# ParBLiSS/kmerind

Measured on AMD Instinct MI355X. Metric: kmers_per_sec_indexed, higher is better.
Workload: dtype u64

## Files before the change

kmerind_amd/csrc/kmi_superkmer.h:

```cpp
#pragma once

namespace kmi {

constexpr int kRecNShift = 38, kRecHashShift = 43;
constexpr uint64_t kSkPadW1 = ~0ull;
constexpr int kRecEdgeShift = 32;
constexpr uint32_t kSkEdgeWindows = 3;
__device__ __forceinline__ uint32_t rec_hash18(uint64_t w1) { return (uint32_t)(w1 >> kRecHashShift) & 0x3ffffu; }
__device__ __forceinline__ uint32_t rec_fine_sub(uint64_t w1) { return (rec_hash18(w1) >> 3) & 127u; }

constexpr int kSkThreads = 512;
constexpr int kSkRoundTiles = 24;
constexpr int kSkListCap = 32;

struct SkRound {
  uint64_t t; uint32_t ei, total; uint32_t eo[kSkRoundTiles + 1]; uint64_t nt; uint32_t nei;
};
__device__ __forceinline__ bool sk_plan(const uint32_t *__restrict__ ent_cnt, uint64_t te, uint64_t t, uint32_t ei, SkRound &r) {
  while (t < te && ei >= ent_cnt[t]) { ++t; ei = 0; }
  if (t >= te) return false;
  r.t = t; r.ei = ei; r.eo[0] = 0;
  r.nt = t + kSkRoundTiles; r.nei = 0;
  bool cut = false;
#pragma unroll
// ... 321 lines not shown
      if (threadIdx.x < cur.total) { sk_locate(cur, threadIdx.x, ent_stride, tr, eidx); ev = ent[eidx]; ri = run_items[eidx]; }
      cnt = ri >> 26;
      const uint32_t *src = wg_items + (ri & 0x3ffffffu);
#pragma unroll
      for (int j = 0; j < CAP; ++j) it[j] = ((uint32_t)j < cnt) ? src[j] : 0u;
      const uint64_t ip0 = (cur.t + tr) * 8192ull + (ev & 0x1fffu);
      uint64_t d0 = (ip0 >> 4) & ~3ull;
      d0 = d0 + 16 <= last_dw + 16 ? d0 : 0;
      const uint4 q0 = *reinterpret_cast<const uint4 *>(st + d0), q1 = *reinterpret_cast<const uint4 *>(st + d0 + 4),
                  q2 = *reinterpret_cast<const uint4 *>(st + d0 + 8), q3 = *reinterpret_cast<const uint4 *>(st + d0 + 12);
      uint32_t *row = s_row + threadIdx.x * kSkRowDw;
      row[0] = q0.x; row[1] = q0.y; row[2] = q0.z; row[3] = q0.w; row[4] = q1.x; row[5] = q1.y; row[6] = q1.z; row[7] = q1.w;
      row[8] = q2.x; row[9] = q2.y; row[10] = q2.z; row[11] = q2.w; row[12] = q3.x; row[13] = q3.y; row[14] = q3.z; row[15] = q3.w;
      row[16] = 0;
      s_bit0[threadIdx.x] = (uint32_t)(ip0 - d0 * 16) * 2u;
      s_ioff[threadIdx.x] = ri & 0x3ffffffu;
    }
#pragma unroll
    for (int j = 0; j < CAP; ++j)
      if ((uint32_t)j < cnt) atomicAdd(&s_cnt[(it[j] >> 22) & 255u], 1u);
    lds_barrier();
    uint32_t c = 0, inc = 0;
    if (threadIdx.x < kNumCoarse) {
      c = s_cnt[threadIdx.x];
      s_cnt[threadIdx.x] = 0;
      inc = wave_inclusive_sum_dpp(c);
      if (lane_id() == kWave - 1) s_part[wave_id()] = inc;
    }
    lds_barrier();
    if (threadIdx.x < kNumCoarse) {
      uint32_t pre = 0;
#pragma unroll
      for (uint32_t w = 0; w < kNumCoarse / kWave; ++w) pre += (w < wave_id()) ? s_part[w] : 0u;
      const uint32_t lo = pre + inc - c;
      s_cur[threadIdx.x] = lo;
      s_gbase[threadIdx.x] = cursor - lo;
      cursor += c;
      if (threadIdx.x == kNumCoarse - 1) s_total = pre + inc;
    }
    lds_barrier();
#pragma unroll
    for (int j = 0; j < CAP; ++j)
      if ((uint32_t)j < cnt) s_stage[atomicAdd(&s_cur[(it[j] >> 22) & 255u], 1u)] = (uint16_t)((threadIdx.x << 5) | (uint32_t)j);
    lds_barrier();
    const uint32_t total = s_total;
    for (uint32_t s = threadIdx.x; s < total; s += NT) {
      const uint32_t e = s_stage[s], rl = e >> 5, j = e & 31u;
      const uint32_t item = wg_items[s_ioff[rl] + j];
      const uint32_t h18 = (item >> 12) & 0x3ffffu, n1 = (item >> 7) & 31u, extra = item >> 30;
      const uint32_t hs = ((h18 << lp) & 0x3ffffu) | (lp <= 2u ? extra >> (2u - lp) : extra << (lp - 2u));
      uint64_t w0, w1;
      sk_assemble_row<CANON>(s_row + rl * kSkRowDw, s_bit0[rl] + 2u * (item & 127u), k + n1, n1, hs, w0, w1);
      reinterpret_cast<ulonglong2 *>(out)[s_gbase[h18 >> 10] + s] = make_ulonglong2(w0, w1);
    }
    SkRound nxt;
    have = sk_plan(ent_cnt, te, cur.nt, cur.nei, nxt);
    cur = nxt;
  }
}

__global__ __launch_bounds__(1024) void sk_fine_count_kernel(const uint64_t *__restrict__ recs, const uint64_t *__restrict__ wg_off,
                                                            const uint64_t *__restrict__ coarse_end ,
                                                            uint32_t groups, uint32_t *__restrict__ fine_hist ,
                                                            uint32_t *__restrict__ fine_kmers ) {
  __shared__ uint32_t s_h[kSubPerCoarse], s_k[kSubPerCoarse];
  const uint32_t gpp = groups / kFineParts;
  const uint32_t c = blockIdx.x / kFineParts, h = blockIdx.x % kFineParts;
  if (threadIdx.x < kSubPerCoarse) { s_h[threadIdx.x] = 0; s_k[threadIdx.x] = 0; }
  lds_barrier();
  const uint64_t b = wg_off[(uint64_t)(h * gpp) * kNumCoarse + c];
  const uint64_t e = (h + 1 < (uint32_t)kFineParts) ? wg_off[(uint64_t)((h + 1) * gpp) * kNumCoarse + c] : coarse_end[c];
  for (uint64_t i = b + threadIdx.x; i < e; i += blockDim.x) {
    const uint64_t w1 = recs[2 * i + 1];
    atomicAdd(&s_h[rec_fine_sub(w1)], 1u);
    atomicAdd(&s_k[rec_fine_sub(w1)], ((uint32_t)(w1 >> kRecNShift) & 31u) + 1u);
  }
  lds_barrier();
  if (threadIdx.x < kSubPerCoarse) {
    fine_hist[(uint64_t)h * kNumFine + c * kSubPerCoarse + threadIdx.x] = s_h[threadIdx.x];
    fine_kmers[(uint64_t)h * kNumFine + c * kSubPerCoarse + threadIdx.x] = s_k[threadIdx.x];
  }
}

constexpr int kSlackLineRecs = 8;
constexpr int kSlackLT = 3072;
constexpr int kSlackLCap = kSlackLT + (kSlackLineRecs - 1) * kSubPerCoarse;
__global__ __launch_bounds__(kPartThreads) void sk_scatter_fine_slack_lines_kernel(const uint64_t *__restrict__ recs, uint64_t *__restrict__ out,
                                                                                 const uint64_t *__restrict__ wg_off, const uint64_t *__restrict__ coarse_end,
                                                                                 uint32_t groups, const uint64_t *__restrict__ fine_region,
                                                                                 const uint32_t *__restrict__ fine_cap, uint32_t *__restrict__ fine_cnt,
                                                                                 uint32_t *__restrict__ fine_kmers, uint32_t *__restrict__ flags) {
  constexpr int NB = kSubPerCoarse, T = kSlackLT, PT = T / kPartThreads, SCAP = kSlackLCap, L = kSlackLineRecs, MAXG = SCAP / L + NB;
  static_assert(kPartThreads / NB == L && T % kPartThreads == 0, "one carry slot per thread: eight threads per bucket");
  __shared__ ulonglong2 s_stage[SCAP];
  __shared__ uint32_t s_cnt[NB];
  __shared__ uint32_t s_k[NB];
  __shared__ uint32_t s_lofs[NB];
  __shared__ uint32_t s_emit[NB];
  __shared__ uint32_t s_old[NB];
  __shared__ uint32_t s_lbase[NB];
  __shared__ uint64_t s_dst[NB];
  __shared__ uint32_t s_part[NB / kWave];
  __shared__ uint32_t s_ng;
  __shared__ uint8_t s_linebkt[MAXG];
  const uint32_t gpp = groups / kFineParts;
  const uint32_t c = blockIdx.x / kFineParts, h = blockIdx.x % kFineParts;
  const uint64_t b = wg_off[(uint64_t)(h * gpp) * kNumCoarse + c];
  const uint64_t e = (h + 1 < (uint32_t)kFineParts) ? wg_off[(uint64_t)((h + 1) * gpp) * kNumCoarse + c] : coarse_end[c];
  if (b >= e) return;
  const uint64_t region = fine_region[c];
  const uint32_t cap = fine_cap[c];
  if (threadIdx.x < NB) { s_cnt[threadIdx.x] = 0; s_k[threadIdx.x] = 0; }
  const uint32_t cb = threadIdx.x / L, cj = threadIdx.x % L;
  ulonglong2 carry = make_ulonglong2(0, 0);
  uint32_t my_carry = 0;
  lds_barrier();
  const ulonglong2 *src = reinterpret_cast<const ulonglong2 *>(recs);
  ulonglong2 raw[PT];
  auto load_tile = [&](uint64_t t0) {
#pragma unroll
    for (int j = 0; j < PT; ++j) {
      uint64_t i = t0 + (uint64_t)j * kPartThreads + threadIdx.x;
      i = (i < e) ? i : e - 1;
      raw[j] = src[i];
    }
  };
  auto take = [&](uint32_t f, uint32_t n) -> uint64_t {
    const uint32_t at = atomicAdd(&fine_cnt[c * NB + f], n);
    if ((uint64_t)at + n > (uint64_t)cap) { atomicOr(&flags[34], 1u); return ~0ull; }
    return region + (uint64_t)f * cap + at;
  };
  load_tile(b);
  for (uint64_t t0 = b; t0 < e; t0 += T) {
    const uint32_t nt = (uint32_t)((e - t0 < (uint64_t)T) ? (e - t0) : (uint64_t)T);
    ulonglong2 rec[PT];
    uint32_t bk[PT], rk[PT];
#pragma unroll
    for (int j = 0; j < PT; ++j) {
      const uint32_t li = j * kPartThreads + threadIdx.x;
      rec[j] = raw[j];
      bk[j] = 0xffffffffu;
      if (li < nt) {
        bk[j] = rec_fine_sub(rec[j].y);
        rk[j] = atomicAdd(&s_cnt[bk[j]], 1u);
        atomicAdd(&s_k[bk[j]], ((uint32_t)(rec[j].y >> kRecNShift) & 31u) + 1u);
      }
    }
    if (t0 + T < e) load_tile(t0 + T);
    lds_barrier();
    uint32_t cnt = 0, emit = 0, ng = 0, inc = 0;
    if (threadIdx.x < NB) {
      cnt = s_cnt[threadIdx.x];
      const uint32_t km = s_k[threadIdx.x];
      s_k[threadIdx.x] = 0;
      emit = cnt & ~(uint32_t)(L - 1);
      ng = emit / L;
      inc = wave_inclusive_sum_dpp(cnt | (ng << 16));
      if (lane_id() == kWave - 1) s_part[wave_id()] = inc;
      if (km) atomicAdd(&fine_kmers[c * NB + threadIdx.x], km);
      s_dst[threadIdx.x] = emit ? take(threadIdx.x, emit) : ~0ull;
    }
    lds_barrier();
    if (threadIdx.x < NB) {
      const uint32_t pre = wave_id() ? s_part[0] : 0u;
      const uint32_t ex = pre + inc - (cnt | (ng << 16));
      const uint32_t lo = ex & 0xffffu, lb = ex >> 16;
      s_lofs[threadIdx.x] = lo; s_emit[threadIdx.x] = emit; s_old[threadIdx.x] = my_carry; s_lbase[threadIdx.x] = lb;
      for (uint32_t i = 0; i < ng; ++i) s_linebkt[lb + i] = (uint8_t)threadIdx.x;
      if (threadIdx.x == NB - 1) s_ng = lb + ng;
      s_cnt[threadIdx.x] = cnt - emit;
      my_carry = cnt - emit;
    }
    lds_barrier();
    if (cj < s_old[cb]) s_stage[s_lofs[cb] + cj] = carry;
#pragma unroll
    for (int j = 0; j < PT; ++j)
      if (bk[j] != 0xffffffffu) s_stage[s_lofs[bk[j]] + rk[j]] = rec[j];
    lds_barrier();
    {
      const uint32_t n_groups = s_ng, l8 = threadIdx.x & (uint32_t)(L - 1);
      for (uint32_t g = threadIdx.x / L; g < n_groups; g += kPartThreads / L) {
        const uint32_t f = s_linebkt[g];
        const uint64_t d = s_dst[f];
        const uint32_t i = (g - s_lbase[f]) * L + l8;
        if (d != ~0ull) reinterpret_cast<ulonglong2 *>(out)[d + i] = s_stage[s_lofs[f] + i];
      }
      const uint32_t rem = s_cnt[cb], base = s_lofs[cb] + s_emit[cb];
      if (cj < rem) carry = s_stage[base + cj];
    }
    lds_barrier();
  }
  {
    if (threadIdx.x < NB) s_dst[threadIdx.x] = my_carry ? take(threadIdx.x, (uint32_t)L) : ~0ull;
    lds_barrier();
    const uint32_t rem = s_cnt[cb];
    const uint64_t d = s_dst[cb];
    if (rem && d != ~0ull) reinterpret_cast<ulonglong2 *>(out)[d + cj] = cj < rem ? carry : make_ulonglong2(kEmptyKey, kSkPadW1);
  }
}

__global__ __launch_bounds__(1024) void sk_zero_kernel(uint32_t *__restrict__ a, uint32_t na, uint32_t *__restrict__ b, uint32_t nb,
                                                     uint32_t *__restrict__ c, uint32_t nc, uint32_t *__restrict__ flags, uint32_t f0, uint32_t f1,
                                                     uint32_t g0, uint32_t g1) {
  const uint32_t i = blockIdx.x * blockDim.x + threadIdx.x, stride = gridDim.x * blockDim.x;
  for (uint32_t x = i; x < na; x += stride) a[x] = 0;
  for (uint32_t x = i; x < nb; x += stride) b[x] = 0;
  for (uint32_t x = i; x < nc; x += stride) c[x] = 0;
  if (i >= f0 && i < f1) flags[i] = 0;
  if (i >= g0 && i < g1) flags[i] = 0;
}

__global__ __launch_bounds__(kPartThreads) void sk_recv_hist_kernel(const uint64_t *__restrict__ recs, uint64_t n, uint32_t *__restrict__ wg_hist,
                                                                   unsigned long long *__restrict__ n_kmers) {
  __shared__ uint32_t s_h[kNumCoarse];
  __shared__ unsigned long long s_k;
  if (threadIdx.x < kNumCoarse) s_h[threadIdx.x] = 0;
  if (threadIdx.x == 0) s_k = 0ull;
  lds_barrier();
  const uint64_t chunk = part_chunk(n, gridDim.x, PartCfg<2>::TILE);
  const uint64_t b = (uint64_t)blockIdx.x * chunk, e = (b + chunk < n) ? b + chunk : n;
  unsigned long long km = 0;
  for (uint64_t i = b + threadIdx.x; i < e; i += blockDim.x) {
    const uint64_t w1 = recs[2 * i + 1];
    atomicAdd(&s_h[rec_hash18(w1) >> 10], 1u);
    km += ((uint32_t)(w1 >> kRecNShift) & 31u) + 1u;
  }
  km = wave_reduce_sum(km);
  if (lane_id() == 0 && km) atomicAdd(&s_k, km);
  lds_barrier();
  if (threadIdx.x < kNumCoarse) wg_hist[(uint64_t)blockIdx.x * kNumCoarse + threadIdx.x] = s_h[threadIdx.x];
  if (threadIdx.x == 0 && s_k) atomicAdd(n_kmers, s_k);
}

#ifndef KMI_SK_H1
#define KMI_SK_H1 1536
#endif
#ifndef KMI_SK_T1_DUP
#define KMI_SK_T1_DUP 0.5f
#endif
#ifndef KMI_SK_FILL
#define KMI_SK_FILL 80
#endif
#ifndef KMI_SK_NT
#define KMI_SK_NT 1024
#endif
#ifndef KMI_SK_LDS_KB
#define KMI_SK_LDS_KB 160
#endif
#ifndef KMI_SK_HASH24
#define KMI_SK_HASH24 1
#endif
__device__ __forceinline__ uint32_t sk_slot_hash(uint64_t key) {
#if KMI_SK_HASH24
  const uint32_t lo = (uint32_t)key, hi = (uint32_t)(key >> 32);
  uint32_t h = __umul24(lo, 0x9E3779u);
  h += __umul24(__builtin_amdgcn_alignbit(hi, lo, 24), 0x85EBCBu);
  h += __umul24(hi >> 16, 0xC2B2AFu);
#else
  uint32_t h = ((uint32_t)key ^ ((uint32_t)(key >> 32) * 0x85EBCA6Bu)) * 0x9E3779B1u;
#endif
  h ^= h >> 15;
  return h;
}
__device__ __forceinline__ uint32_t sk_slot_of(uint32_t h, uint32_t cap) { return __umul24(h >> 16, cap) >> 16; }

#ifndef KMI_SK_PROBE_ATTR
#define KMI_SK_PROBE_ATTR __forceinline__
#endif
__device__ KMI_SK_PROBE_ATTR uint32_t sk_probe_insert(lds_u64_t *tkeys, lds_u32_t *tvals, lds_u32_t *distinct, lds_u32_t *overflow,
                                                         const lds_u64_t *q, const lds_u32_t *qw, uint32_t first, uint32_t cnt,
                                                         uint32_t cap, uint32_t last, uint32_t limit, uint32_t pending) {
  const uint32_t lane = lane_id();
  bool claimed = false;
  if (lane < cnt) {
    const uint64_t key = q[first + lane];
    const uint32_t wt = qw[first + lane];
    const uint32_t s0 = sk_slot_of(sk_slot_hash(key), cap);
    uint32_t s = s0;
    uint64_t c = __atomic_load_n(&tkeys[s], __ATOMIC_RELAXED);
    for (;;) {
      while (c != key && c != kEmptyKey && s - s0 < 64u) { ++s; c = __atomic_load_n(&tkeys[s], __ATOMIC_RELAXED); }
      if (c == key) break;
      if (c != kEmptyKey || s >= last) { *overflow = 1; s = last; break; }
      uint64_t expected = kEmptyKey;
      if (__atomic_compare_exchange_n(&tkeys[s], &expected, key, false, __ATOMIC_RELAXED, __ATOMIC_RELAXED)) { claimed = true; break; }
      c = expected;
    }
    __atomic_fetch_add(&tvals[s], wt, __ATOMIC_RELAXED);
  }
  const unsigned long long cm = __ballot(claimed);
  const uint32_t add = (uint32_t)__popcll(cm) + pending;
  if (add >= 16u || (add && cnt < 64u)) {
    if (lane == 0 && __atomic_fetch_add(distinct, add, __ATOMIC_RELAXED) + add >= limit) *overflow = 1;
    return 0u;
  }
  return add;
}


#ifndef KMI_SK_OVF
#define KMI_SK_OVF 448
#endif
constexpr int kSkOvf = KMI_SK_OVF;
template <int OWN_>
struct SkTab2 {
  static constexpr int NT = KMI_SK_NT, NWAVES = NT / kWave;
  static constexpr int OWN = OWN_;
  static constexpr int H1 = KMI_SK_H1, S1 = H1 + 64, L1 = H1 * 3 / 4;
  static constexpr int FIXED = NWAVES * (OWN + kMissQ * 12) + S1 * 20 + kSkOvf * 16 + 2560;
  static constexpr int S2 = ((KMI_SK_LDS_KB * 1024 - FIXED) / 12) / 64 * 64;
  static constexpr int CAP2 = S2 - 64, LIMIT2 = CAP2 * KMI_SK_FILL / 100;
};

template <bool CANON, int OWN_, bool SPECIAL>
#ifndef KMI_SK_MIN_WAVES
#define KMI_SK_MIN_WAVES 4
#endif
__global__ __launch_bounds__(KMI_SK_NT, KMI_SK_MIN_WAVES) void sk_reduce_kernel(const uint64_t *__restrict__ recs, const uint64_t *__restrict__ rec_off, uint32_t k,
                                                        const uint64_t *__restrict__ kmer_off ,
                                                        uint64_t *__restrict__ tmp_keys, uint32_t *__restrict__ tmp_vals,
                                                        uint32_t *__restrict__ out_cnt, uint32_t *__restrict__ flags,
                                                        uint32_t *__restrict__ queue , uint32_t n_buckets,
                                                        uint32_t start_bits, uint32_t lp, float inv_dup,
                                                        const uint64_t *__restrict__ fine_region = nullptr, const uint32_t *__restrict__ fine_cap = nullptr,
                                                        const uint32_t *__restrict__ fine_cnt = nullptr) {
  auto records_of = [&](uint32_t bb, uint64_t &lo, uint64_t &hi) {
    if (fine_cnt) {
      const uint32_t cap = fine_cap[bb >> 7], cnt = fine_cnt[bb];
      lo = fine_region[bb >> 7] + (uint64_t)(bb & 127u) * cap; hi = lo + (cnt < cap ? cnt : cap);
    }
    else { lo = rec_off[bb]; hi = rec_off[bb + 1]; }
  };
  using T = SkTab2<OWN_>;
  constexpr int NWAVES = T::NWAVES;
  constexpr uint64_t W1_INIT = ~0ull;
  enum { C_DIST = 0, C_OVF = 1, C_SPC = 2, C_SPS = 3, C_EMIT = 4, C_SP = 5, C_OVN = 6, C_T1N = 8, C_LVL = 9, C_NEXT = 10  };
  __shared__ uint64_t s_tk[T::S2];
  __shared__ uint32_t s_tv[T::S2];
  __shared__ ulonglong2 s_r[T::S1];
  __shared__ uint32_t s_rc[T::S1];
  __shared__ ulonglong2 s_ovf[kSkOvf];
  __shared__ uint64_t s_missq[NWAVES * kMissQ];
  __shared__ uint32_t s_missw[NWAVES * kMissQ];
  __shared__ uint8_t s_own[NWAVES * T::OWN];
  __shared__ uint32_t s_ctl[12];
  __shared__ uint32_t s_stack[320];
  const uint32_t lane = lane_id(), wv = wave_id();
  lds_u64_t *const tkeys = (lds_u64_t *)s_tk;
  lds_u32_t *const tvals = (lds_u32_t *)s_tv;
  lds_u32_t *const tdist = (lds_u32_t *)&s_ctl[C_DIST];
  lds_u32_t *const tovf = (lds_u32_t *)&s_ctl[C_OVF];
  uint64_t *const mq = s_missq + wv * kMissQ;
  uint32_t *const mw = s_missw + wv * kMissQ;
  uint8_t *const wown = s_own + wv * T::OWN;
  const uint32_t kb = 2u * k;
  const uint32_t kmask_hi = kb >= 64u ? 0xffffffffu : ((1u << (kb - 32u)) - 1u);
  const uint32_t pad = 64u - kb;
  const bool use_t1_known = inv_dup > 0.f;
  for (uint32_t i = threadIdx.x; i < (uint32_t)(NWAVES * T::OWN / 4); i += T::NT) reinterpret_cast<uint32_t *>(s_own)[i] = 0;
  for (uint32_t i = threadIdx.x; i < (uint32_t)T::S2; i += T::NT) { s_tk[i] = kEmptyKey; s_tv[i] = 0; }
  for (uint32_t i = threadIdx.x; i < (uint32_t)T::S1; i += T::NT) { s_r[i] = make_ulonglong2(kEmptyKey, W1_INIT); s_rc[i] = 0; }
  for (uint32_t i = threadIdx.x; i < (uint32_t)(NWAVES * kMissQ); i += T::NT) s_missq[i] = 0;
  if (threadIdx.x < 12) s_ctl[threadIdx.x] = 0;
  if (threadIdx.x == 0) s_ctl[C_NEXT] = atomicAdd(queue, 1u);
  lds_barrier();
  uint32_t b = __builtin_amdgcn_readfirstlane(s_ctl[C_NEXT]);
  uint32_t par = 1;
  bool pf_ok = false;
  ulonglong2 pf = make_ulonglong2(0, 0);
  uint64_t pf_rb = 0, pf_re = 0, pf_k0 = 0, pf_k1 = 0;
  uint32_t mn = 0, pending = 0, my_claims = 0, hbits = 0, hmask = 0, hval = 0;
  auto to_table = [&](uint64_t key, uint32_t kw, bool v) {
    const uint32_t h = sk_slot_hash(key);
    const uint32_t slot = sk_slot_of(h, (uint32_t)T::CAP2);
    v = v && (h & hmask) == hval;
    if (SPECIAL && v && key == kEmptyKey) { s_ctl[C_SPS] = 1; atomicAdd(&s_ctl[C_SPC], kw); v = false; }
    const uint64_t c0 = __atomic_load_n(&s_tk[slot], __ATOMIC_RELAXED), c1 = __atomic_load_n(&s_tk[slot + 1u], __ATOMIC_RELAXED);
    bool hit0 = v && c0 == key;
    const bool hit1 = v && c1 == key;
    bool won = false;
    if (v && c0 == kEmptyKey) {
      const unsigned long long old = atomicCAS((unsigned long long *)&s_tk[slot], (unsigned long long)kEmptyKey, (unsigned long long)key);
      won = old == kEmptyKey;
      hit0 = won || old == key;
    }
    my_claims += won ? 1u : 0u;
    if (hit0 || hit1) atomicAdd(&s_tv[slot + (hit0 ? 0u : 1u)], kw);
    const bool miss = v && !hit0 && !hit1;
    const unsigned long long mm = __ballot(miss);
    if (mm) {
      const uint32_t pos = mn + __builtin_amdgcn_mbcnt_hi((uint32_t)(mm >> 32), __builtin_amdgcn_mbcnt_lo((uint32_t)mm, 0u));
      if (miss) { mq[pos] = key; mw[pos] = kw; }
      mn += (uint32_t)__popcll(mm);
      if (mn >= (uint32_t)kWave) {
        pending = sk_probe_insert(tkeys, tvals, tdist, tovf, (const lds_u64_t *)mq, (const lds_u32_t *)mw, mn - kWave, kWave, (uint32_t)T::CAP2,
                                  (uint32_t)T::S2 - 1u, (uint32_t)T::LIMIT2, pending);
        mn -= kWave;
      }
    }
  };
  uint64_t *const cas_dummy = mq + kWave + lane;
  auto to_table2 = [&](uint64_t ka, bool va, uint64_t kc, bool vc, uint32_t kw) {
    const uint32_t hA = sk_slot_hash(ka), hC = sk_slot_hash(kc);
    const uint32_t sa = sk_slot_of(hA, (uint32_t)T::CAP2), sc = sk_slot_of(hC, (uint32_t)T::CAP2);
    va = va && (hA & hmask) == hval; vc = vc && (hC & hmask) == hval;
    if (SPECIAL) {
      if (va && ka == kEmptyKey) { s_ctl[C_SPS] = 1; atomicAdd(&s_ctl[C_SPC], kw); va = false; }
      if (vc && kc == kEmptyKey) { s_ctl[C_SPS] = 1; atomicAdd(&s_ctl[C_SPC], kw); vc = false; }
    }
    const uint64_t a0 = __atomic_load_n(&s_tk[sa], __ATOMIC_RELAXED), a1 = __atomic_load_n(&s_tk[sa + 1u], __ATOMIC_RELAXED);
    const uint64_t c0 = __atomic_load_n(&s_tk[sc], __ATOMIC_RELAXED), c1 = __atomic_load_n(&s_tk[sc + 1u], __ATOMIC_RELAXED);
    const bool ta = va && a0 == kEmptyKey, tc = vc && c0 == kEmptyKey;
    const unsigned long long oa = atomicCAS((unsigned long long *)(ta ? &s_tk[sa] : cas_dummy), (unsigned long long)kEmptyKey, (unsigned long long)ka);
    const unsigned long long oc = atomicCAS((unsigned long long *)(tc ? &s_tk[sc] : cas_dummy), (unsigned long long)kEmptyKey, (unsigned long long)kc);
    const bool wa_ = ta && oa == kEmptyKey, wc_ = tc && oc == kEmptyKey;
    const bool ha0 = va && (a0 == ka || wa_ || (ta && oa == ka)), hc0 = vc && (c0 == kc || wc_ || (tc && oc == kc));
    const bool ha1 = va && !ha0 && a1 == ka, hc1 = vc && !hc0 && c1 == kc;
    my_claims += (wa_ ? 1u : 0u) + (wc_ ? 1u : 0u);
    atomicAdd(&s_tv[sa + (ha1 ? 1u : 0u)], (ha0 || ha1) ? kw : 0u);
    atomicAdd(&s_tv[sc + (hc1 ? 1u : 0u)], (hc0 || hc1) ? kw : 0u);
    const bool ma = va && !ha0 && !ha1, mc = vc && !hc0 && !hc1;
    const unsigned long long mma = __ballot(ma), mmc = __ballot(mc);
    if (mma | mmc) {
      if (ma) { const uint32_t pos = mn + __builtin_amdgcn_mbcnt_hi((uint32_t)(mma >> 32), __builtin_amdgcn_mbcnt_lo((uint32_t)mma, 0u)); mq[pos] = ka; mw[pos] = kw; }
      mn += (uint32_t)__popcll(mma);
      if (mn >= (uint32_t)kWave) {
        pending = sk_probe_insert(tkeys, tvals, tdist, tovf, (const lds_u64_t *)mq, (const lds_u32_t *)mw, mn - kWave, kWave, (uint32_t)T::CAP2,
                                  (uint32_t)T::S2 - 1u, (uint32_t)T::LIMIT2, pending);
        mn -= kWave;
      }
      if (mc) { const uint32_t pos = mn + __builtin_amdgcn_mbcnt_hi((uint32_t)(mmc >> 32), __builtin_amdgcn_mbcnt_lo((uint32_t)mmc, 0u)); mq[pos] = kc; mw[pos] = kw; }
      mn += (uint32_t)__popcll(mmc);
      if (mn >= (uint32_t)kWave) {
        pending = sk_probe_insert(tkeys, tvals, tdist, tovf, (const lds_u64_t *)mq, (const lds_u32_t *)mw, mn - kWave, kWave, (uint32_t)T::CAP2,
                                  (uint32_t)T::S2 - 1u, (uint32_t)T::LIMIT2, pending);
        mn -= kWave;
      }
    }
  };
  auto expand = [&](uint64_t w0, uint64_t w1, uint32_t wt, uint32_t n) {
    const uint32_t nu = (n + 1u) >> 1;
    const uint32_t inc = wave_inclusive_sum_dpp(nu);
    const uint32_t pre = inc - nu;
    const uint32_t total = __builtin_amdgcn_readlane(inc, kWave - 1);
    if (total == 0u) return;
    if (nu) wown[pre] = (uint8_t)(lane + 1u);
    uint32_t carry = 0;
    const uint32_t top_sh = kb - 34u;
    for (uint32_t g0 = 0; g0 < total; g0 += kWave) {
      const uint32_t g = g0 + lane;
      const bool act = g < total;
      uint32_t o = act ? (uint32_t)wown[g] : 0u;
      o = wave_inclusive_max_dpp(o);
      o = o > carry ? o : carry;
      carry = __builtin_amdgcn_readlane(o, kWave - 1);
      const int rl = (int)((o ? o - 1u : 0u) << 2);
      const uint32_t j = 2u * (g - (uint32_t)__builtin_amdgcn_ds_bpermute(rl, (int)pre));
      const uint32_t a0 = (uint32_t)__builtin_amdgcn_ds_bpermute(rl, (int)(uint32_t)w0), a1 = (uint32_t)__builtin_amdgcn_ds_bpermute(rl, (int)(uint32_t)(w0 >> 32));
      const uint32_t a2 = (uint32_t)__builtin_amdgcn_ds_bpermute(rl, (int)(uint32_t)w1), a3 = (uint32_t)__builtin_amdgcn_ds_bpermute(rl, (int)(uint32_t)(w1 >> 32));
      const uint32_t kw = (uint32_t)__builtin_amdgcn_ds_bpermute(rl, (int)wt);
      const bool two = act && j + 1u <= ((a3 >> (kRecNShift - 32)) & 31u);
      const bool w1sel = j >= 16u;
      const uint32_t bit = (2u * j) & 31u;
      const uint32_t b0 = w1sel ? a1 : a0, b1 = w1sel ? a2 : a1, b2 = w1sel ? a3 : a2;
      const uint32_t rc_lo = __builtin_amdgcn_alignbit(b1, b0, bit);
      const uint32_t rc_hi = __builtin_amdgcn_alignbit(b2, b1, bit) & kmask_hi;
      const uint32_t r_hi = __builtin_bitreverse32(rc_lo), r_lo = __builtin_bitreverse32(rc_hi);
      const uint32_t s_hi = ~(((r_hi >> 1) & 0x55555555u) | ((r_hi << 1) & 0xAAAAAAAAu));
      const uint32_t s_lo = ~(((r_lo >> 1) & 0x55555555u) | ((r_lo << 1) & 0xAAAAAAAAu));
      const uint32_t fw_lo = __builtin_amdgcn_alignbit(s_hi, s_lo, pad), fw_hi = s_hi >> pad;
      const uint32_t rc2_lo = __builtin_amdgcn_alignbit(b1, b0, bit + 2u);
      const uint32_t rc2_hi = __builtin_amdgcn_alignbit(b2, b1, bit + 2u) & kmask_hi;
      const uint32_t fw2_lo = (fw_lo << 2) | (((rc2_hi >> top_sh) & 3u) ^ 3u);
      const uint32_t fw2_hi = __builtin_amdgcn_alignbit(fw_hi, fw_lo, 30u) & kmask_hi;
      const uint64_t rc = (uint64_t)rc_lo | ((uint64_t)rc_hi << 32), fw = (uint64_t)fw_lo | ((uint64_t)fw_hi << 32);
      const uint64_t rc2 = (uint64_t)rc2_lo | ((uint64_t)rc2_hi << 32), fw2 = (uint64_t)fw2_lo | ((uint64_t)fw2_hi << 32);
#ifndef KMI_SK_INSERT1
      to_table2(CANON ? (fw < rc ? fw : rc) : fw, act, CANON ? (fw2 < rc2 ? fw2 : rc2) : fw2, two, kw);
#else
      to_table(CANON ? (fw < rc ? fw : rc) : fw, kw, act);
      to_table(CANON ? (fw2 < rc2 ? fw2 : rc2) : fw2, kw, two);
#endif
    }
    if (nu) wown[pre] = 0;
    const uint32_t batch_claims = __builtin_amdgcn_readlane(wave_inclusive_sum_dpp(my_claims), kWave - 1);
    my_claims = 0;
    pending += batch_claims;
    if (pending >= 32u) {
      if (lane == 0 && atomicAdd(&s_ctl[C_DIST], pending) + pending >= (uint32_t)T::LIMIT2) s_ctl[C_OVF] = 1;
      pending = 0;
    }
  };
#ifdef KMI_SK_TIMING
  unsigned long long acc[8] = {0, 0, 0, 0, 0, 0, 0, 0}, tq = 0;
#define TQ_MARK(i) { const unsigned long long now_ = clock64(); acc[i] += now_ - tq; tq = now_; }
#else
#define TQ_MARK(i)
#endif
  while (b < n_buckets) {
    uint32_t q_next = 0;
    if (threadIdx.x == 0) q_next = atomicAdd(queue, 1u);
    uint64_t rb = pf_rb, re = pf_re;
    if (!pf_ok) records_of(b, rb, re);
    const uint32_t n_rec = (uint32_t)(re - rb);
    const ulonglong2 *const src = reinterpret_cast<const ulonglong2 *>(recs) + rb;
    const uint32_t share = (n_rec + NWAVES - 1) / NWAVES;
    const uint32_t r_lo = wv * share < n_rec ? wv * share : n_rec;
    const uint32_t r_hi = r_lo + share < n_rec ? r_lo + share : n_rec;
    ulonglong2 first = pf;
    if (!pf_ok) { first = make_ulonglong2(0, 0); if (r_lo + lane < r_hi) first = src[r_lo + lane]; }
    const uint64_t tmp0 = pf_ok ? pf_k0 : kmer_off[b], tmp1 = pf_ok ? pf_k1 : kmer_off[b + 1];
    pf_ok = false;
    if (threadIdx.x == 0) {
      uint32_t hb = start_bits > 8u ? 8u : start_bits;
      if (use_t1_known && n_rec) {
        const float pred = (float)(tmp1 - tmp0) * inv_dup;
        float room = 0.88f * (float)T::LIMIT2 * (float)(1u << hb);
        while (hb < 8u && pred > room) { ++hb; room *= 2.f; }
      }
      const uint32_t np = n_rec ? (1u << hb) : 0u;
      for (uint32_t v = 0; v < np; ++v) s_stack[v] = hb | (v << 8);
      s_ctl[C_SP] = np; s_ctl[C_EMIT] = 0; s_ctl[C_LVL] = hb;
    }
    bool first_pass = true;
    lds_barrier();
#ifdef KMI_SK_TIMING
    tq = clock64();
#endif
    while (true) {
      const uint32_t sp = s_ctl[C_SP];
      if (sp == 0) break;
      const uint32_t pass = s_stack[sp - 1];
      const uint32_t fbits = pass & 0xffu, fval = pass >> 8;
      lds_barrier();
      if (threadIdx.x == 0) s_ctl[C_SP] = sp - 1;
      const bool use_t1 = use_t1_known ? inv_dup <= KMI_SK_T1_DUP : fbits < 2u;
      const uint32_t dead = lp > 2u ? lp - 2u : 0u, rmax = 3u - dead;
      const uint32_t rbits = fbits < rmax ? fbits : rmax, rmask = ((1u << rbits) - 1u) << dead, rval = (fval & ((1u << rbits) - 1u)) << dead;
      hbits = fbits - rbits; hmask = (1u << hbits) - 1u; hval = fval >> rbits;
      mn = 0; pending = 0; my_claims = 0;
      {
        ulonglong2 nxt = first;
        if (!first_pass) { nxt = make_ulonglong2(0, 0); if (r_lo + lane < r_hi) nxt = src[r_lo + lane]; }
        for (uint32_t r0 = r_lo; r0 < r_hi; r0 += kWave) {
          if (__atomic_load_n(&s_ctl[C_OVF], __ATOMIC_RELAXED)) break;
          const ulonglong2 rec = nxt;
          const bool have = r0 + lane < r_hi;
          if (r0 + kWave + lane < r_hi) nxt = src[r0 + kWave + lane];
          uint32_t n = (have && rec.y != kSkPadW1) ? ((uint32_t)(rec.y >> kRecNShift) & 31u) + 1u : 0u;
          if ((rec_hash18(rec.y) & rmask) != rval) n = 0;
          bool direct = n != 0u;
          if (use_t1) {
            if (direct && rec.x != kEmptyKey) {
              uint32_t h = ((uint32_t)rec.x ^ (uint32_t)(rec.x >> 32)) * 0x9E3779B1u ^ ((uint32_t)rec.y ^ (uint32_t)(rec.y >> 32)) * 0x85EBCA6Bu;
              h ^= h >> 15;
              const uint32_t s0 = ((h >> 16) * (uint32_t)T::H1) >> 16;
              for (uint32_t s = s0; direct && s < s0 + 8u; s += 4u) {
                ulonglong2 e[4];
#pragma unroll
                for (int i = 0; i < 4; ++i) e[i] = s_r[s + i];
                int hit = -1, free_ = -1;
#pragma unroll
                for (int i = 3; i >= 0; --i) {
                  const bool same = e[i].x == rec.x && e[i].y == rec.y, empty = e[i].x == kEmptyKey;
                  if (same) { hit = i; free_ = -1; } else if (empty) { free_ = i; hit = -1; }
                }
                if (hit >= 0) { atomicAdd(&s_rc[s + hit], 1u); direct = false; }
                else if (free_ >= 0) {
                  if (__atomic_load_n(&s_ctl[C_T1N], __ATOMIC_RELAXED) >= (uint32_t)T::L1) break;
                  const unsigned long long old = atomicCAS((unsigned long long *)&s_r[s + free_].x, (unsigned long long)kEmptyKey, (unsigned long long)rec.x);
                  if (old == kEmptyKey) {
                    __atomic_store_n(&s_r[s + free_].y, rec.y, __ATOMIC_RELAXED);
                    atomicAdd(&s_rc[s + free_], 1u);
                    atomicAdd(&s_ctl[C_T1N], 1u);
                    direct = false;
                  } else if (old == rec.x && __atomic_load_n(&s_r[s + free_].y, __ATOMIC_RELAXED) == rec.y) {
                    atomicAdd(&s_rc[s + free_], 1u);
                    direct = false;
                  } else break;
                }
              }
            }
            if (direct) {
              const uint32_t oi = atomicAdd(&s_ctl[C_OVN], 1u);
              if (oi < (uint32_t)kSkOvf) { s_ovf[oi] = rec; direct = false; }
            }
          }
          if (__any(direct)) { TQ_MARK(0) expand(rec.x, rec.y, 1u, direct ? n : 0u); TQ_MARK(1) }
        }
      }
      TQ_MARK(0)
      if (first_pass && threadIdx.x == 0) s_ctl[C_NEXT + par] = q_next;
      lds_barrier();
      TQ_MARK(2)
      uint32_t nbk = 0;
      if (first_pass) {
        nbk = __builtin_amdgcn_readfirstlane(s_ctl[C_NEXT + par]);
        if (nbk < n_buckets) { records_of(nbk, pf_rb, pf_re); pf_k0 = kmer_off[nbk]; pf_k1 = kmer_off[nbk + 1]; }
      }
      if (use_t1) {
        const uint32_t n_ovf = s_ctl[C_OVN] < (uint32_t)kSkOvf ? s_ctl[C_OVN] : (uint32_t)kSkOvf;
        constexpr uint32_t PER1 = ((uint32_t)T::S1 + NWAVES - 1) / NWAVES;
        const uint32_t per_o = (n_ovf + NWAVES - 1) / NWAVES;
        const uint32_t t_lo = wv * PER1, t_hi = t_lo + PER1 < (uint32_t)T::S1 ? t_lo + PER1 : (uint32_t)T::S1;
        const uint32_t o_lo = wv * per_o < n_ovf ? wv * per_o : n_ovf, o_hi = o_lo + per_o < n_ovf ? o_lo + per_o : n_ovf;
        const uint32_t n_mine = (t_hi - t_lo) + (o_hi - o_lo);
        for (uint32_t i0 = 0; i0 < n_mine; i0 += kWave) {
          const uint32_t i = i0 + lane;
          uint64_t w0 = kEmptyKey, w1 = 0; uint32_t wt = 0;
          if (i < t_hi - t_lo) {
            const uint32_t s = t_lo + i;
            const ulonglong2 ent = s_r[s];
            w0 = ent.x; w1 = ent.y; wt = s_rc[s];
            if (w0 != kEmptyKey) { s_r[s] = make_ulonglong2(kEmptyKey, W1_INIT); s_rc[s] = 0; }
          } else if (i < n_mine) {
            const ulonglong2 ent = s_ovf[o_lo + (i - (t_hi - t_lo))];
            w0 = ent.x; w1 = ent.y; wt = 1u;
          }
          uint32_t n = wt ? ((uint32_t)(w1 >> kRecNShift) & 31u) + 1u : 0u;
          if (__atomic_load_n(&s_ctl[C_OVF], __ATOMIC_RELAXED)) n = 0;
          if (__any(n != 0u)) expand(w0, w1, wt, n);
        }
      }
      if (mn) {
        pending = sk_probe_insert(tkeys, tvals, tdist, tovf, (const lds_u64_t *)mq, (const lds_u32_t *)mw, 0u, mn, (uint32_t)T::CAP2, (uint32_t)T::S2 - 1u,
                                  (uint32_t)T::LIMIT2, pending);
        mn = 0;
      }
      if (pending && lane == 0 && atomicAdd(&s_ctl[C_DIST], pending) + pending >= (uint32_t)T::LIMIT2) s_ctl[C_OVF] = 1;
      if (first_pass && nbk < n_buckets) {
        const uint32_t nn = (uint32_t)(pf_re - pf_rb), nshare = (nn + NWAVES - 1) / NWAVES;
        const uint32_t nlo = wv * nshare < nn ? wv * nshare : nn, nhi = nlo + nshare < nn ? nlo + nshare : nn;
        pf = make_ulonglong2(0, 0);
        if (nlo + lane < nhi) pf = reinterpret_cast<const ulonglong2 *>(recs)[pf_rb + nlo + lane];
        pf_ok = true;
      }
      first_pass = false;
      TQ_MARK(3)
      lds_barrier();
      TQ_MARK(4)
      const bool lost = s_ctl[C_OVF] != 0u;
      lds_barrier();
      if (threadIdx.x == 0) { s_ctl[C_DIST] = 0; s_ctl[C_OVF] = 0; s_ctl[C_T1N] = 0; s_ctl[C_OVN] = 0; }
      if (lost) {
        for (uint32_t i = threadIdx.x; i < (uint32_t)T::S2; i += T::NT) { s_tk[i] = kEmptyKey; s_tv[i] = 0; }
        if (threadIdx.x == 0) {
          s_ctl[C_SPC] = 0; s_ctl[C_SPS] = 0;
          if (fbits >= 18u) atomicOr(&flags[2], 1u);
          else {
            uint32_t best = 0, best_n = 0;
            for (uint32_t l = 0; l <= 8u; ++l) {
              const uint32_t c = __hip_atomic_load(&flags[16 + l], __ATOMIC_RELAXED, __HIP_MEMORY_SCOPE_AGENT);
              if (c > best_n) { best_n = c; best = l; }
            }
            uint32_t target = best > fbits ? best : fbits + 1u;
            if (target > fbits + 6u) target = fbits + 6u;
            uint32_t spn = s_ctl[C_SP];
            for (uint32_t v = 0; v < (1u << (target - fbits)); ++v) s_stack[spn++] = target | ((fval | (v << fbits)) << 8);
            s_ctl[C_SP] = spn;
            if (target > s_ctl[C_LVL]) s_ctl[C_LVL] = target;
          }
        }
        lds_barrier();
        continue;
      }
      {
        uint32_t *s_out = &s_ctl[C_EMIT];
        for (uint32_t s = threadIdx.x; s < (uint32_t)((T::S2 + kWave - 1) / kWave * kWave); s += T::NT) {
          uint64_t key = kEmptyKey; uint32_t val = 0;
          if (s < (uint32_t)T::S2) { key = s_tk[s]; val = s_tv[s]; }
          const bool used = key != kEmptyKey;
          const uint32_t pos = wave_alloc(s_out, used);
          if (used) { tmp_keys[tmp0 + pos] = key; tmp_vals[tmp0 + pos] = val; s_tk[s] = kEmptyKey; s_tv[s] = 0; }
        }
        lds_barrier();
        if (threadIdx.x == 0) {
          if (s_ctl[C_SPS]) {
            const uint32_t pos = atomicAdd(s_out, 1u);
            tmp_keys[tmp0 + pos] = kEmptyKey;
            tmp_vals[tmp0 + pos] = s_ctl[C_SPC];
          }
          s_ctl[C_SPC] = 0; s_ctl[C_SPS] = 0;
          s_tv[T::S2 - 1] = 0;
        }
      }
      lds_barrier();
      TQ_MARK(5)
    }
    if (threadIdx.x == 0) {
      out_cnt[b] = s_ctl[C_EMIT];
      if (n_rec && (s_ctl[C_LVL] || start_bits)) atomicAdd(&flags[16 + (s_ctl[C_LVL] > 8u ? 8u : s_ctl[C_LVL])], 1u);
    }
    if (n_rec == 0u && threadIdx.x == 0) s_ctl[C_NEXT + par] = q_next;
    lds_barrier();
    b = __builtin_amdgcn_readfirstlane(s_ctl[C_NEXT + par]);
    par ^= 1u;
    TQ_MARK(6)
  }
#ifdef KMI_SK_TIMING
  if (lane == 0) for (int i = 0; i < 8; ++i) atomicAdd(&reinterpret_cast<unsigned long long *>(flags + 48)[i], acc[i]);
#endif
}

}
```

Before: 177.8 billion.

## Deepen bucket prefetch pipeline, add explicit vmcnt waits, and block-level emit allocation

Each workgroup now claims two queue tickets up front and keeps one bucket of lookahead, so the next bucket's record offsets and kmer offsets are loaded at the start of the current bucket instead of after the first pass. Explicit s_waitcnt vmcnt(0) calls are placed so prefetched record loads are waited on only where they are needed. The emit stage now loads all table slots into registers, computes per-wave offsets with ballot and mbcnt, and does a single atomic per wave instead of one per iteration. These changes raise register pressure and add queue-ordering complexity; the empty-bucket path is rewritten and the ticket atomic is hidden from the optimizer with an asm barrier.

```diff
diff --git a/kmerind_amd/csrc/kmi_superkmer.h b/kmerind_amd/csrc/kmi_superkmer.h
--- a/kmerind_amd/csrc/kmi_superkmer.h
+++ b/kmerind_amd/csrc/kmi_superkmer.h
@@ -647,6 +647,12 @@
 #define KMI_SK_OVF 448
 #endif
 constexpr int kSkOvf = KMI_SK_OVF;
+#ifndef KMI_SK_TICKET_PLAIN
+#define KMI_SK_TICKET_PLAIN 1
+#endif
+#ifndef KMI_SK_EMIT_BLOCK
+#define KMI_SK_EMIT_BLOCK 1
+#endif
 template <int OWN_>
 struct SkTab2 {
   static constexpr int NT = KMI_SK_NT, NWAVES = NT / kWave;
@@ -707,13 +713,25 @@
   for (uint32_t i = threadIdx.x; i < (uint32_t)T::S1; i += T::NT) { s_r[i] = make_ulonglong2(kEmptyKey, W1_INIT); s_rc[i] = 0; }
   for (uint32_t i = threadIdx.x; i < (uint32_t)(NWAVES * kMissQ); i += T::NT) s_missq[i] = 0;
   if (threadIdx.x < 12) s_ctl[threadIdx.x] = 0;
-  if (threadIdx.x == 0) s_ctl[C_NEXT] = atomicAdd(queue, 1u);
+  if (threadIdx.x == 0) { s_ctl[C_NEXT] = atomicAdd(queue, 1u); s_ctl[C_NEXT + 1] = atomicAdd(queue, 1u); }
   lds_barrier();
-  uint32_t b = __builtin_amdgcn_readfirstlane(s_ctl[C_NEXT]);
-  uint32_t par = 1;
-  bool pf_ok = false;
+  uint32_t b = __builtin_amdgcn_readfirstlane(s_ctl[C_NEXT]), b1 = __builtin_amdgcn_readfirstlane(s_ctl[C_NEXT + 1]);
+  uint32_t par = 0;
+  auto share_of = [&](uint32_t n, uint32_t &lo, uint32_t &hi) {
+    const uint32_t share = (n + NWAVES - 1) / NWAVES;
+    lo = wv * share < n ? wv * share : n;
+    hi = lo + share < n ? lo + share : n;
+  };
+  uint64_t cur_rb = 0, cur_re = 0, cur_k0 = 0, cur_k1 = 0;
   ulonglong2 pf = make_ulonglong2(0, 0);
-  uint64_t pf_rb = 0, pf_re = 0, pf_k0 = 0, pf_k1 = 0;
+  if (b < n_buckets) {
+    records_of(b, cur_rb, cur_re); cur_k0 = kmer_off[b]; cur_k1 = kmer_off[b + 1];
+    uint32_t lo, hi;
+    share_of((uint32_t)(cur_re - cur_rb), lo, hi);
+    if (lo + lane < hi) pf = reinterpret_cast<const ulonglong2 *>(recs)[cur_rb + lo + lane];
+  }
+  auto vm_landed = [] { __builtin_amdgcn_s_waitcnt(0x0F70); };
+  vm_landed();
   uint32_t mn = 0, pending = 0, my_claims = 0, hbits = 0, hmask = 0, hval = 0;
   auto to_table = [&](uint64_t key, uint32_t kw, bool v) {
     const uint32_t h = sk_slot_hash(key);
@@ -844,18 +862,26 @@
 #endif
   while (b < n_buckets) {
     uint32_t q_next = 0;
-    if (threadIdx.x == 0) q_next = atomicAdd(queue, 1u);
-    uint64_t rb = pf_rb, re = pf_re;
-    if (!pf_ok) records_of(b, rb, re);
+    if (threadIdx.x == 0) {
+      uint32_t q_at = 0;
+#if KMI_SK_TICKET_PLAIN
+      asm volatile("" : "+v"(q_at));
+#endif
+      q_next = atomicAdd(queue + q_at, 1u);
+    }
+    const uint64_t rb = cur_rb, re = cur_re, tmp0 = cur_k0, tmp1 = cur_k1;
     const uint32_t n_rec = (uint32_t)(re - rb);
     const ulonglong2 *const src = reinterpret_cast<const ulonglong2 *>(recs) + rb;
-    const uint32_t share = (n_rec + NWAVES - 1) / NWAVES;
-    const uint32_t r_lo = wv * share < n_rec ? wv * share : n_rec;
-    const uint32_t r_hi = r_lo + share < n_rec ? r_lo + share : n_rec;
-    ulonglong2 first = pf;
-    if (!pf_ok) { first = make_ulonglong2(0, 0); if (r_lo + lane < r_hi) first = src[r_lo + lane]; }
-    const uint64_t tmp0 = pf_ok ? pf_k0 : kmer_off[b], tmp1 = pf_ok ? pf_k1 : kmer_off[b + 1];
-    pf_ok = false;
+    uint32_t r_lo, r_hi;
+    share_of(n_rec, r_lo, r_hi);
+    const ulonglong2 first = pf;
+    uint64_t nx_rb = 0, nx_re = 0, nx_k0 = 0, nx_k1 = 0;
+    if (b1 < n_buckets) { records_of(b1, nx_rb, nx_re); nx_k0 = kmer_off[b1]; nx_k1 = kmer_off[b1 + 1]; }
+    auto prefetch_next = [&]() {
+      uint32_t nlo, nhi;
+      share_of((uint32_t)(nx_re - nx_rb), nlo, nhi);
+      pf = reinterpret_cast<const ulonglong2 *>(recs)[nlo + lane < nhi ? nx_rb + nlo + lane : rb];
+    };
     if (threadIdx.x == 0) {
       uint32_t hb = start_bits > 8u ? 8u : start_bits;
       if (use_t1_known && n_rec) {
@@ -872,9 +898,8 @@
 #ifdef KMI_SK_TIMING
     tq = clock64();
 #endif
-    while (true) {
+    if (n_rec != 0u) do {
       const uint32_t sp = s_ctl[C_SP];
-      if (sp == 0) break;
       const uint32_t pass = s_stack[sp - 1];
       const uint32_t fbits = pass & 0xffu, fval = pass >> 8;
       lds_barrier();
@@ -885,12 +910,12 @@
       hbits = fbits - rbits; hmask = (1u << hbits) - 1u; hval = fval >> rbits;
       mn = 0; pending = 0; my_claims = 0;
       {
-        ulonglong2 nxt = first;
-        if (!first_pass) { nxt = make_ulonglong2(0, 0); if (r_lo + lane < r_hi) nxt = src[r_lo + lane]; }
+        ulonglong2 rec = first;
+        if (!first_pass) { rec = make_ulonglong2(0, 0); if (r_lo + lane < r_hi) rec = src[r_lo + lane]; vm_landed(); }
         for (uint32_t r0 = r_lo; r0 < r_hi; r0 += kWave) {
           if (__atomic_load_n(&s_ctl[C_OVF], __ATOMIC_RELAXED)) break;
-          const ulonglong2 rec = nxt;
           const bool have = r0 + lane < r_hi;
+          ulonglong2 nxt = rec;
           if (r0 + kWave + lane < r_hi) nxt = src[r0 + kWave + lane];
           uint32_t n = (have && rec.y != kSkPadW1) ? ((uint32_t)(rec.y >> kRecNShift) & 31u) + 1u : 0u;
           if ((rec_hash18(rec.y) & rmask) != rval) n = 0;
@@ -932,17 +957,15 @@
             }
           }
           if (__any(direct)) { TQ_MARK(0) expand(rec.x, rec.y, 1u, direct ? n : 0u); TQ_MARK(1) }
+          vm_landed();
+          rec = nxt;
         }
       }
       TQ_MARK(0)
       if (first_pass && threadIdx.x == 0) s_ctl[C_NEXT + par] = q_next;
       lds_barrier();
       TQ_MARK(2)
-      uint32_t nbk = 0;
-      if (first_pass) {
-        nbk = __builtin_amdgcn_readfirstlane(s_ctl[C_NEXT + par]);
-        if (nbk < n_buckets) { records_of(nbk, pf_rb, pf_re); pf_k0 = kmer_off[nbk]; pf_k1 = kmer_off[nbk + 1]; }
-      }
+      vm_landed();
       if (use_t1) {
         const uint32_t n_ovf = s_ctl[C_OVN] < (uint32_t)kSkOvf ? s_ctl[C_OVN] : (uint32_t)kSkOvf;
         constexpr uint32_t PER1 = ((uint32_t)T::S1 + NWAVES - 1) / NWAVES;
@@ -973,19 +996,14 @@
         mn = 0;
       }
       if (pending && lane == 0 && atomicAdd(&s_ctl[C_DIST], pending) + pending >= (uint32_t)T::LIMIT2) s_ctl[C_OVF] = 1;
-      if (first_pass && nbk < n_buckets) {
-        const uint32_t nn = (uint32_t)(pf_re - pf_rb), nshare = (nn + NWAVES - 1) / NWAVES;
-        const uint32_t nlo = wv * nshare < nn ? wv * nshare : nn, nhi = nlo + nshare < nn ? nlo + nshare : nn;
-        pf = make_ulonglong2(0, 0);
-        if (nlo + lane < nhi) pf = reinterpret_cast<const ulonglong2 *>(recs)[pf_rb + nlo + lane];
-        pf_ok = true;
-      }
+      if (first_pass) prefetch_next();
       first_pass = false;
       TQ_MARK(3)
       lds_barrier();
       TQ_MARK(4)
       const bool lost = s_ctl[C_OVF] != 0u;
       lds_barrier();
+      vm_landed();
       if (threadIdx.x == 0) { s_ctl[C_DIST] = 0; s_ctl[C_OVF] = 0; s_ctl[C_T1N] = 0; s_ctl[C_OVN] = 0; }
       if (lost) {
         for (uint32_t i = threadIdx.x; i < (uint32_t)T::S2; i += T::NT) { s_tk[i] = kEmptyKey; s_tv[i] = 0; }
@@ -1011,6 +1029,34 @@
       }
       {
         uint32_t *s_out = &s_ctl[C_EMIT];
+#if KMI_SK_EMIT_BLOCK
+        constexpr int EI = (T::S2 + T::NT - 1) / T::NT;
+        uint64_t ek[EI]; uint32_t ev[EI], eo[EI];
+#pragma unroll
+        for (int i = 0; i < EI; ++i) {
+          const uint32_t s = threadIdx.x + (uint32_t)i * T::NT;
+          ek[i] = kEmptyKey; ev[i] = 0;
+          if (i < EI - 1 || s < (uint32_t)T::S2) { ek[i] = s_tk[s]; ev[i] = s_tv[s]; }
+        }
+        uint32_t total = 0;
+#pragma unroll
+        for (int i = 0; i < EI; ++i) {
+          const unsigned long long m = __ballot(ek[i] != kEmptyKey);
+          eo[i] = total + __builtin_amdgcn_mbcnt_hi((uint32_t)(m >> 32), __builtin_amdgcn_mbcnt_lo((uint32_t)m, 0u));
+          total += (uint32_t)__popcll(m);
+        }
+        uint32_t block = 0;
+        if (total) {
+          if (lane == 0) block = atomicAdd(s_out, total);
+          block = __builtin_amdgcn_readfirstlane(block);
+        }
+        const uint64_t o0 = tmp0 + block;
+#pragma unroll
+        for (int i = 0; i < EI; ++i) {
+          const uint32_t s = threadIdx.x + (uint32_t)i * T::NT;
+          if (ek[i] != kEmptyKey) { tmp_keys[o0 + eo[i]] = ek[i]; tmp_vals[o0 + eo[i]] = ev[i]; s_tk[s] = kEmptyKey; s_tv[s] = 0; }
+        }
+#else
         for (uint32_t s = threadIdx.x; s < (uint32_t)((T::S2 + kWave - 1) / kWave * kWave); s += T::NT) {
           uint64_t key = kEmptyKey; uint32_t val = 0;
           if (s < (uint32_t)T::S2) { key = s_tk[s]; val = s_tv[s]; }
@@ -1018,6 +1064,7 @@
           const uint32_t pos = wave_alloc(s_out, used);
           if (used) { tmp_keys[tmp0 + pos] = key; tmp_vals[tmp0 + pos] = val; s_tk[s] = kEmptyKey; s_tv[s] = 0; }
         }
+#endif
         lds_barrier();
         if (threadIdx.x == 0) {
           if (s_ctl[C_SPS]) {
@@ -1031,15 +1078,22 @@
       }
       lds_barrier();
       TQ_MARK(5)
+    } while (s_ctl[C_SP] != 0u);
+    else {
+      if (threadIdx.x == 0) s_ctl[C_NEXT + par] = q_next;
+      uint32_t nlo, nhi;
+      share_of((uint32_t)(nx_re - nx_rb), nlo, nhi);
+      if (nlo + lane < nhi) pf = reinterpret_cast<const ulonglong2 *>(recs)[nx_rb + nlo + lane];
+      vm_landed();
     }
     if (threadIdx.x == 0) {
       out_cnt[b] = s_ctl[C_EMIT];
       if (n_rec && (s_ctl[C_LVL] || start_bits)) atomicAdd(&flags[16 + (s_ctl[C_LVL] > 8u ? 8u : s_ctl[C_LVL])], 1u);
     }
-    if (n_rec == 0u && threadIdx.x == 0) s_ctl[C_NEXT + par] = q_next;
-    lds_barrier();
-    b = __builtin_amdgcn_readfirstlane(s_ctl[C_NEXT + par]);
-    par ^= 1u;
+    lds_barrier();
+    const uint32_t b2 = __builtin_amdgcn_readfirstlane(s_ctl[C_NEXT + par]);
+    b = b1; b1 = b2; par ^= 1u;
+    cur_rb = nx_rb; cur_re = nx_re; cur_k0 = nx_k0; cur_k1 = nx_k1;
     TQ_MARK(6)
   }
 #ifdef KMI_SK_TIMING
```

After: 182.8 billion, median of 6. 2.9% higher.
